# microsoft/DirectXTex

Measured on AMD Instinct MI355X. Metric: Mtexels/s BC7 encode (4096^2 RGBA8, TEX_COMPRESS_DEFAULT), higher is better.
Workload: dtype fp32 seed fit + i32 exact error sums (u8 texels in, 128-bit blocks out); 1 GPU; cfg2: 4096x4096 RGBA8 -> BC7_UNORM, TEX_COMPRESS_DEFAULT, one image per GPU, source and payload resident in HBM (dxtex_compress_device)

## Files before the change

### directxtex_amd/csrc/bc6h_encode.hip

```cpp
#include "dxtex_kernels.h"
#include "bc67_tables.h"
#include "bc7_core.h"
#include "bc6h_core.h"
#include "search_common.h"
#include <algorithm>
#include <cstdlib>
#include <cstdio>
#include <vector>

namespace dxtex
{
namespace
{
using namespace bc6h;

struct Ep16 { uint32_t a01, a2b0, b12; };
__device__ __forceinline__ Ep16 pack_ep16(const int (&A)[3], const int (&B)[3])
{
    Ep16 e;
    e.a01 = (uint32_t(A[0]) & 0xFFFFu) | (uint32_t(A[1]) << 16);
    e.a2b0 = (uint32_t(A[2]) & 0xFFFFu) | (uint32_t(B[0]) << 16);
    e.b12 = (uint32_t(B[1]) & 0xFFFFu) | (uint32_t(B[2]) << 16);
    return e;
}
// ... 973 lines not shown
        if (lane == 0) idx = atomicAdd(head, 1u);
        idx = uint32_t(__builtin_amdgcn_readfirstlane(int(idx)));
        if (idx >= live) break;
        const uint32_t myTask = a.order[idx].x;
        const Rec6 rec = a.recs[myTask];
        const uint32_t nb = myTask % a.nblocks;
        const int prec = a.prec1[myTask / a.nblocks];
        const float* gp = a.fpix + uint64_t(nb) * 48 + (lane & 15);
        const float tr = gp[0], tg = gp[16], tb = gp[32];
        EndPts e;
        unpack_ep16(rec.ep, sg, e.A, e.B);
        Perturb6 st = perturb6_begin(e, rec.err);
        while (st.ch < 3)
        {
            float err; int v;
            perturb6_wave_macro(tr, tg, tb, lane, st, prec, sg, err, v);
            st = perturb6_transition(st, err, v);
        }
        if (lane == 0)
        {
            a.recs[myTask].ep = pack_ep16(st.ep.A, st.ep.B);
            { const float mk = ep16_mark(sg, st.ep.A, st.ep.B); if (mk < 0.0f) a.recs[myTask].err = mk; }
        }
    }
}

__global__ void __launch_bounds__(256) bc6h_store_kernel(Bc6hArgs a)
{
    const uint32_t nb = blockIdx.x * 256u + threadIdx.x;
    if (nb >= a.nblocks) return;
    const Best6 b = a.best[nb];
    const BcSeg& im = seg_of(a.seg, nb);
    const uint32_t gb = im.nb0 + (nb - im.l0);
    const uint32_t by = gb / im.nbw, bx = gb - by * im.nbw;
    uint64_t* out = reinterpret_cast<uint64_t*>(im.dst + uint64_t(by) * im.dstRowPitch) + 2 * uint64_t(bx);
    out[0] = b.lo; out[1] = b.hi;
}

const uint64_t kMaxBlocksPerPass6 = dev_env("DXTEX_MAX_BLOCKS_PER_PASS") ? std::max<uint64_t>(1, strtoull(dev_env("DXTEX_MAX_BLOCKS_PER_PASS"), nullptr, 10)) : (1u << 22);
struct Scratch6
{
    size_t fpix, lists, seeds, recs, orgs, order, tinfo, counters, best, bounds, recs1, orgs1, order1, tinfo1, counters1, opts, total;
    explicit Scratch6(uint64_t nb)
    {
        auto up = [](size_t v) { return (v + 255) & ~size_t(255); };
        size_t o = 0;
        fpix = o; o = up(o + nb * 48 * sizeof(float));
        lists = o; o = up(o + nb * 8);
        seeds = o; o = up(o + nb * SEED_INTS * sizeof(int));
        recs = o; o = up(o + nb * 16 * sizeof(Rec6));
        orgs = o; o = up(o + nb * 16 * sizeof(OrgSave));
        order = o; o = up(o + nb * 16 * sizeof(uint2));
        tinfo = o; o = up(o + nb * 16 * sizeof(uint32_t));
        counters = o; o = up(o + 128 * sizeof(uint32_t));
        best = o; o = up(o + nb * sizeof(Best6));
        bounds = o; o = up(o + nb * 17 * sizeof(float));
        recs1 = o; o = up(o + nb * 4 * sizeof(Rec6));
        orgs1 = o; o = up(o + nb * 4 * sizeof(OrgSave));
        order1 = o; o = up(o + nb * 4 * sizeof(uint2));
        tinfo1 = o; o = up(o + nb * 4 * sizeof(uint32_t));
        counters1 = o; o = up(o + 128 * sizeof(uint32_t));
        opts = o; o = up(o + nb * 16 * sizeof(OptSave));
        total = o;
    }
};
}

size_t bc6h_scratch_bytes(uint64_t nblocks, size_t nimages)
{
    return Scratch6(nblocks < kMaxBlocksPerPass6 ? nblocks : kMaxBlocksPerPass6).total + seg_table_bytes(nblocks, kMaxBlocksPerPass6, nimages);
}

hipError_t launch_bc6h_encode(const SrcView& src, uint8_t* dst, uint64_t dstRowPitch, bool isSigned, void* scratch,
                              hipStream_t stream, KernelMarks* marks, const SideStreams* side)
{
    BcImage one; one.src = src; one.dst = dst; one.dstRowPitch = dstRowPitch;
    return launch_bc6h_encode_many(&one, 1, isSigned, scratch, stream, marks, side);
}

hipError_t launch_bc6h_encode_many(const BcImage* images, size_t count, bool isSigned, void* scratch, hipStream_t stream, KernelMarks* marks,
                                   const SideStreams* side)
{
#define DXTEX_MARK(NAME) do { if (marks) marks->mark(NAME); } while (0)
    std::vector<BcSeg> segs;
    std::vector<BcPass> passes;
    uint64_t perPass = 0;
    if (!build_passes(images, count, kMaxBlocksPerPass6, segs, passes, &perPass)) return hipSuccess;
    const Scratch6 L(perPass);
    uint8_t* base = static_cast<uint8_t*>(scratch);
    BcSeg* dSegs = reinterpret_cast<BcSeg*>(base + L.total);
    const hipError_t ce = upload_segments(dSegs, segs, passes, stream);
    if (ce != hipSuccess) return ce;
    for (const BcPass& pass : passes)
    {
        Bc6hArgs a;
        set_pass(a.seg, dSegs, segs, pass);
        a.nblocks = pass.nblocks;
        a.isSigned = isSigned ? 1 : 0;
        static const bool noPrune = dev_env("DXTEX_BC6H_NO_PRUNE") != nullptr;
        a.prune = noPrune ? 0 : 1;
        a.fpix = reinterpret_cast<float*>(base + L.fpix);
        a.lists = base + L.lists;
        a.seeds = reinterpret_cast<int*>(base + L.seeds);
        a.recs = reinterpret_cast<Rec6*>(base + L.recs);
        a.orgs = reinterpret_cast<OrgSave*>(base + L.orgs);
        a.order = reinterpret_cast<uint2*>(base + L.order);
        a.tinfo = reinterpret_cast<uint32_t*>(base + L.tinfo);
        a.counters = reinterpret_cast<uint32_t*>(base + L.counters);
        a.best = reinterpret_cast<Best6*>(base + L.best);
        a.bounds = reinterpret_cast<float*>(base + L.bounds);
        a.opts = reinterpret_cast<OptSave*>(base + L.opts);
        a.saveOpt = 0;
        a.boundsReady = 0;
        a.filterStats = 0;
        a.mode = ModeRt();

        DXTEX_MARK("bc6h_rough");
        hipLaunchKernelGGL(bc6h_rough_kernel, dim3((a.nblocks + 3) / 4), dim3(256), 0, stream, a);
        DXTEX_MARK("bc6h_block_seed");
        hipLaunchKernelGGL(bc6h_block_seed_kernel, dim3((a.nblocks + 255) / 256), dim3(256), 0, stream, a);
        if (dev_env("DXTEX_BC6H_DUMP"))
        {
            (void)hipStreamSynchronize(stream);
            const uint32_t n = std::min<uint32_t>(a.nblocks, 4);
            std::vector<uint8_t> l(n * 8); std::vector<int> sd(n * SEED_INTS);
            (void)hipMemcpy(l.data(), a.lists, l.size(), hipMemcpyDeviceToHost);
            (void)hipMemcpy(sd.data(), a.seeds, sd.size() * 4, hipMemcpyDeviceToHost);
            for (uint32_t b = 0; b < n; ++b)
            {
                fprintf(stderr, "block %u shapes:", b);
                for (int i = 0; i < 8; ++i) fprintf(stderr, " %d", l[b * 8 + i]);
                fprintf(stderr, "\n  seeds rank0:");
                for (int i = 0; i < 12; ++i) fprintf(stderr, " %d", sd[b * SEED_INTS + i]);
                fprintf(stderr, "\n");
            }
        }
        static const int onlyMode = dev_env("DXTEX_BC6H_ONLY_MODE") ? atoi(dev_env("DXTEX_BC6H_ONLY_MODE")) : -1;
        static const bool noSearch = dev_env("DXTEX_BC6H_NO_SEARCH") != nullptr;
        static const Bc6hMode kModes[14] = {
            { 0x00, 1, 1, 3, { 10, 10, 10 }, { 5, 5, 5 } }, { 0x01, 1, 1, 3, { 7, 7, 7 }, { 6, 6, 6 } }, { 0x02, 1, 1, 3, { 11, 11, 11 }, { 5, 4, 4 } },
            { 0x06, 1, 1, 3, { 11, 11, 11 }, { 4, 5, 4 } }, { 0x0a, 1, 1, 3, { 11, 11, 11 }, { 4, 4, 5 } }, { 0x0e, 1, 1, 3, { 9, 9, 9 }, { 5, 5, 5 } },
            { 0x12, 1, 1, 3, { 8, 8, 8 }, { 6, 5, 5 } }, { 0x16, 1, 1, 3, { 8, 8, 8 }, { 5, 6, 5 } }, { 0x1a, 1, 1, 3, { 8, 8, 8 }, { 5, 5, 6 } },
            { 0x1e, 1, 0, 3, { 6, 6, 6 }, { 6, 6, 6 } }, { 0x03, 0, 0, 4, { 10, 10, 10 }, { 10, 10, 10 } }, { 0x07, 0, 1, 4, { 11, 11, 11 }, { 9, 9, 9 } },
            { 0x0b, 0, 1, 4, { 12, 12, 12 }, { 8, 8, 8 } }, { 0x0f, 0, 1, 4, { 16, 16, 16 }, { 4, 4, 4 } } };
        auto set_mode_on = [&](Bc6hArgs& a, int mi)
        {
            const Bc6hMode& k = kModes[mi];
            a.mode.index = mi; a.mode.code = k.code; a.mode.regions2 = k.regions2; a.mode.transformed = k.transformed; a.mode.prec = k.prec[0];
            for (int c = 0; c < 3; ++c) a.mode.delta[c] = k.delta[c];
        };
        auto set_mode = [&](int mi) { set_mode_on(a, mi); };
        auto sort_tasks = [&](const Bc6hArgs& a, uint32_t ntasks, hipStream_t stream)
        {
            const uint32_t binGroups = std::min<uint32_t>(kBinGroups, (ntasks + 255) / 256);
            (void)hipMemsetAsync(a.counters, 0, 128 * sizeof(uint32_t), stream);
            hipLaunchKernelGGL(bc7_bin_count_kernel, dim3(binGroups), dim3(256), 0, stream, a.tinfo, ntasks, a.counters);
            hipLaunchKernelGGL(bc7_bin_scan_kernel, dim3(1), dim3(1), 0, stream, a.counters);
            hipLaunchKernelGGL(bc7_bin_scatter_kernel, dim3(binGroups), dim3(256), 0, stream, a.tinfo, ntasks, a.counters, a.order);
        };
        a.taskBase = 0;
        for (int m = 0; m < 4; ++m) a.prec1[m] = kModes[10 + m].prec[0];
        static const std::vector<int> order6 = []
        {
            std::vector<int> o;
            const char* e = dev_env("DXTEX_BC6H_ORDER");
            const char* p = e ? e : DXTEX_BC6H_DEFAULT_ORDER;
            while (*p) { if (*p >= '0' && *p <= '9') o.push_back(int(strtol(p, const_cast<char**>(&p), 10))); else ++p; }
            return o;
        }();
        int prevPrec = -1;
        a.samePrec = 0;
        std::vector<int> run2;
        for (int mi : order6) if (mi >= 0 && mi <= 9 && (onlyMode < 0 || mi == onlyMode)) run2.push_back(mi);
        static const int forkBack = dev_env("DXTEX_BC6H_FORK_BACK") ? atoi(dev_env("DXTEX_BC6H_FORK_BACK")) : 2;
        const SideStreams* fork = (marks || forkBack <= 0 || run2.size() < size_t(forkBack) + 1 || onlyMode >= 0) ? nullptr : side;
        Bc6hArgs a1 = a;
        a1.recs = reinterpret_cast<Rec6*>(base + L.recs1);
        a1.orgs = reinterpret_cast<OrgSave*>(base + L.orgs1);
        a1.order = reinterpret_cast<uint2*>(base + L.order1);
        a1.tinfo = reinterpret_cast<uint32_t*>(base + L.tinfo1);
        a1.counters = reinterpret_cast<uint32_t*>(base + L.counters1);
        a1.samePrec = 0;
        auto one_region_search = [&](hipStream_t stream, KernelMarks* marks)
        {
            const uint32_t gridPP = (a1.nblocks + 255) / 256;
            DXTEX_MARK("bc6h_pre_1region");
            a1.boundsReady = 0;
            for (int m = 0; m < 4; ++m)
            {
                if (onlyMode >= 0 && 10 + m != onlyMode) continue;
                set_mode_on(a1, 10 + m); a1.taskBase = uint32_t(m) * a1.nblocks;
                hipLaunchKernelGGL(bc6h_pre_kernel<0>, dim3(gridPP), dim3(256), 0, stream, a1);
                a1.boundsReady = 1;
            }
            const uint32_t ntasks = a1.nblocks * 4u;
            if (onlyMode >= 0)
                for (int m = 0; m < 4; ++m) if (10 + m != onlyMode) (void)hipMemsetAsync(a1.tinfo + uint64_t(m) * a1.nblocks, 0, uint64_t(a1.nblocks) * 4, stream);
            DXTEX_MARK("bc6h_bin_1region");
            sort_tasks(a1, ntasks, stream);
            DXTEX_MARK("bc6h_perturb_1region");
            static const uint32_t waveMax = dev_env("DXTEX_BC6H_WAVE_MAX") ? uint32_t(strtoul(dev_env("DXTEX_BC6H_WAVE_MAX"), nullptr, 0)) : kWaveTaskMax6;
            if (!noSearch)
            {
                hipLaunchKernelGGL(bc6h_perturb_kernel<16>, dim3(std::min<uint32_t>(kSearchWaves, (ntasks + 63) / 64)), dim3(64), 0, stream, a1, waveMax);
                hipLaunchKernelGGL(bc6h_perturb_wave_kernel, dim3(std::min<uint32_t>(kSearchWaves, ntasks)), dim3(64), 0, stream, a1, waveMax);
            }
        };
        bool forked = false;
        for (size_t at = 0; at < run2.size(); ++at)
        {
            const int mi = run2[at];
// ... 87 lines not shown
```

### directxtex_amd/csrc/bc7_encode.hip

```cpp
#include "dxtex_kernels.h"
#include "bc67_tables.h"
#include "bc7_core.h"
#include "search_common.h"
#include <algorithm>
#include <cstdio>
#include <cstdlib>
#include <vector>

namespace dxtex
{
namespace
{
using namespace bc7;

struct Cand { uint32_t err; uint32_t ord; uint64_t lo, hi; };

enum : int { SLOT_M0 = 0, SLOT_M1, SLOT_M2, SLOT_M3, SLOT_M4A, SLOT_M4B, SLOT_M5, SLOT_M6, SLOT_M7, NUM_SLOTS };
enum : int { LIST_BYTES = 64 };

enum : int { PHASE_ALL = 0, PHASE_EARLY = 1, PHASE_LATE = 2 };

struct Bc7Args
{
    SegTable seg;
// ... 1244 lines not shown
    const BcSeg& sg = seg_of(a.seg, i >> 4);
    load_block_texel(sg.src, sg.nbw, sg.nb0 + ((i >> 4) - sg.l0), i & 15u, f4, ldr);
    a.px[i] = ldr;
    if ((i & 15u) == 0) { a.zeroOrd[i >> 4] = 0xFFFFFFFFu; a.bestErr[i >> 4] = 0x7FFFFFFF; }
}

__global__ void __launch_bounds__(256) bc7_pick_kernel(Bc7Args a, uint32_t slotMask)
{
    const uint32_t nb = blockIdx.x * 256u + threadIdx.x;
    if (nb >= a.nblocks) return;
    const Cand* c = a.cands + uint64_t(nb) * NUM_SLOTS;
    uint64_t bestKey = ~0ull;
    uint64_t lo = 0, hi = 0;
#pragma unroll
    for (int s = 0; s < NUM_SLOTS; ++s)
    {
        if (!((slotMask >> s) & 1u)) continue;
        if (s == SLOT_M7 && a.flagged[1] == 0) continue;
        const Cand v = c[s];
        if (v.err == 0xFFFFFFFFu) continue;
        const uint64_t key = (uint64_t(v.err) << 32) | v.ord;
        if (key < bestKey) { bestKey = key; lo = v.lo; hi = v.hi; }
    }
    const BcSeg& sg = seg_of(a.seg, nb);
    const uint32_t gb = sg.nb0 + (nb - sg.l0);
    const uint32_t by = gb / sg.nbw, bx = gb - by * sg.nbw;
    uint64_t* out = reinterpret_cast<uint64_t*>(sg.dst + uint64_t(by) * sg.dstRowPitch) + 2 * uint64_t(bx);
    out[0] = lo; out[1] = hi;
}
}

namespace
{
const uint64_t kMaxBlocksPerPass = dev_env("DXTEX_MAX_BLOCKS_PER_PASS") ? std::max<uint64_t>(1, strtoull(dev_env("DXTEX_MAX_BLOCKS_PER_PASS"), nullptr, 10)) : (1u << 22);
constexpr int kMaxTasksPerBlock = 64;
const uint64_t kSmallPassBlocks = dev_env("DXTEX_BC7_SMALL_BLOCKS") ? strtoull(dev_env("DXTEX_BC7_SMALL_BLOCKS"), nullptr, 10) : 262144;
struct ScratchLayout
{
    size_t lists, cands, px, recs, order, tinfo, counters, zeroOrd, bestErr, seeds, seeds1, seeds3, flagcnt, auxRecs, auxOrder, auxTinfo, auxCounters, total;
    size_t auxTpb, auxSlices;
    explicit ScratchLayout(uint64_t nb, bool threeSubsets)
    {
        auto up = [](size_t v) { return (v + 255) & ~size_t(255); };
        const size_t tpb = threeSubsets ? kMaxTasksPerBlock : 32;
        const bool small = nb <= kSmallPassBlocks;
        auxTpb = small ? tpb : 4; auxSlices = small ? size_t(kSideStreams) : 2;
        size_t o = 0;
        lists = o; o = up(o + nb * LIST_BYTES);
        cands = o; o = up(o + nb * NUM_SLOTS * sizeof(Cand));
        px = o; o = up(o + nb * 64);
        recs = o; o = up(o + nb * tpb * sizeof(TaskRec));
        order = o; o = up(o + nb * tpb * sizeof(uint2));
        tinfo = o; o = up(o + nb * tpb * sizeof(uint32_t));
        counters = o; o = up(o + 64 * sizeof(uint32_t));
        zeroOrd = o; o = up(o + nb * sizeof(uint32_t));
        bestErr = o; o = up(o + nb * sizeof(int));
        seeds = o; o = up(o + nb * 64 * sizeof(uint2));
        seeds1 = o; o = up(o + nb * 2 * sizeof(uint2));
        seeds3 = o; o = up(o + (threeSubsets ? nb * 192 * sizeof(uint2) : 0));
        flagcnt = o; o = up(o + 256);
        auxRecs = o; o = up(o + auxSlices * nb * auxTpb * sizeof(TaskRec));
        auxOrder = o; o = up(o + auxSlices * nb * auxTpb * sizeof(uint2));
        auxTinfo = o; o = up(o + auxSlices * nb * auxTpb * sizeof(uint32_t));
        auxCounters = o; o = up(o + size_t(kSideStreams) * 64 * sizeof(uint32_t));
        total = o;
    }
};

template<int MODE, int IM>
void launch_mode(const Bc7Args& a0, hipStream_t stream, KernelMarks* marks, const char* const (&names)[7])
{
    typedef TaskMap<MODE, IM> TM;
    constexpr int BPW = (TM::TPB >= 64) ? 1 : 64 / TM::TPB;
    const uint32_t nb = a0.nblocks;
    const uint32_t ntasks = nb * uint32_t(TM::TPB);
    const uint32_t gridPP = (nb + 4 * BPW - 1) / (4 * BPW);
    constexpr bool kWhole = TM::NS == 1;
    constexpr uint32_t kExhMax = (MODE == 6) ? kWaveTaskMax : kWaveTaskMax45;
    static const bool noGroup = dev_env("DXTEX_BC7_NO_GROUP") != nullptr;
    const bool maybeShortP = kWhole && !noGroup && (MODE == 6 || ntasks <= 4u * kPerturbWaveMax);
    const bool maybeShortE = kWhole && !noGroup && (MODE == 6 || ntasks <= 4u * kExhMax);
    const uint32_t wavesP = std::min<uint32_t>(kSearchWaves, (ntasks + 1) / 2), wavesE = std::min<uint32_t>(kSearchWaves, ntasks);
    Bc7Args a = a0;
    a.gate = nullptr; a.gateMin = 0;
    if (a0.flagged && !(a0.flags & BCF_BC7_QUICK))
    {
        if (MODE == 7) { a.gate = a0.flagged + 1; a.gateMin = 1; }
        else if (a0.phase == PHASE_EARLY && (MODE == 4 || MODE == 5)) { a.gate = a0.flagged + 1; a.gateMin = std::max<uint32_t>(1u, a0.earlyAlphaMin); }
        else if (a0.phase == PHASE_EARLY && MODE == 6) { a.gate = a0.flagged; a.gateMin = std::max<uint32_t>(1u, a0.early6Min); }
    }
    a.perturbWaveMax = maybeShortP ? kPerturbWaveMax : 0u;
    a.exhWaveMax = maybeShortE ? kExhMax : 0u;
    if (marks) marks->mark(names[0]);
    hipLaunchKernelGGL((bc7_pre_kernel<MODE, IM>), dim3(gridPP), dim3(256), 0, stream, a);
    if (marks) marks->mark(names[1]);
    (void)hipMemsetAsync(a.counters, 0, 64 * sizeof(uint32_t), stream);
    const uint32_t binGroups = std::min<uint32_t>(kBinGroups, (ntasks + 255) / 256);
    hipLaunchKernelGGL(bc7_bin_count_kernel, dim3(binGroups), dim3(256), 0, stream, a.tinfo, ntasks, a.counters, a.gate, a.gateMin);
    hipLaunchKernelGGL(bc7_bin_scan_kernel, dim3(1), dim3(1), 0, stream, a.counters);
    hipLaunchKernelGGL(bc7_bin_scatter_kernel, dim3(binGroups), dim3(256), 0, stream, a.tinfo, ntasks, a.counters, a.order, a.gate, a.gateMin);
    if (marks) marks->mark(names[2]);
    const uint32_t waves = std::min<uint32_t>(kSearchWaves, (ntasks + 63) / 64);
    static const int tailBelow = dev_env("DXTEX_BC7_TAIL_BELOW") ? atoi(dev_env("DXTEX_BC7_TAIL_BELOW")) : 48;
    static const bool perturbPlain = dev_env("DXTEX_BC7_PERTURB_PLAIN") != nullptr;
    static const int rangeTests = dev_env("DXTEX_BC7_NO_PEEL") ? 3 : ((dev_env("DXTEX_BC7_RANGE_TESTS") ? atoi(dev_env("DXTEX_BC7_RANGE_TESTS")) & 0xFF : DXTEX_RANGE_TESTS) |
                                                                       ((dev_env("DXTEX_BC7_PEEL_LAYERS") ? atoi(dev_env("DXTEX_BC7_PEEL_LAYERS")) : 1) << 8));
    if constexpr (PaletteBits<MODE, IM>::AB == 0)
    {
        if constexpr (MODE == 1 || MODE == 6)
        {
            if (perturbPlain) hipLaunchKernelGGL((bc7_perturb_kernel<MODE, IM, CH_ALL>), dim3(waves), dim3(64), 0, stream, a, 0);
            else hipLaunchKernelGGL((bc7_perturb_filter_kernel<MODE, IM, CH_ALL>), dim3(waves), dim3(64), 0, stream, a, 0);
        }
        else
            hipLaunchKernelGGL((bc7_perturb_kernel<MODE, IM, CH_ALL>), dim3(waves), dim3(64), 0, stream, a, 0);
        if constexpr (kWhole) { if (maybeShortP) hipLaunchKernelGGL((bc7_perturb_wave_kernel<MODE, IM, CH_ALL>), dim3(wavesP), dim3(64), 0, stream, a); }
        if (marks) marks->mark(names[4]);
        if constexpr (kWhole) { if (maybeShortE) hipLaunchKernelGGL((bc7_exhaustive_wave_kernel<MODE, IM, CH_ALL>), dim3(wavesE), dim3(64), 0, stream, a); }
        hipLaunchKernelGGL((bc7_exhaustive_kernel<MODE, IM, CH_ALL>), dim3(waves), dim3(64), 0, stream, a, 1, tailBelow, rangeTests);
    }
    else
    {
        if constexpr (MODE == 4 && IM == 1 && DXTEX_PF_M4 != 0)
        {
            if (perturbPlain) hipLaunchKernelGGL((bc7_perturb_kernel<MODE, IM, CH_COLOR>), dim3(waves), dim3(64), 0, stream, a, 0);
            else hipLaunchKernelGGL((bc7_perturb_filter_kernel<MODE, IM, CH_COLOR>), dim3(waves), dim3(64), 0, stream, a, 0);
        }
        else
            hipLaunchKernelGGL((bc7_perturb_kernel<MODE, IM, CH_COLOR>), dim3(waves), dim3(64), 0, stream, a, 0);
        if (maybeShortP) hipLaunchKernelGGL((bc7_perturb_wave_kernel<MODE, IM, CH_COLOR>), dim3(wavesP), dim3(64), 0, stream, a);
        if (marks) marks->mark(names[3]);
        hipLaunchKernelGGL((bc7_perturb_kernel<MODE, IM, CH_ALPHA>), dim3(waves), dim3(64), 0, stream, a, 1);
        if (maybeShortP) hipLaunchKernelGGL((bc7_perturb_wave_kernel<MODE, IM, CH_ALPHA>), dim3(wavesP), dim3(64), 0, stream, a);
        if (marks) marks->mark(names[4]);
        if (maybeShortE) hipLaunchKernelGGL((bc7_exhaustive_wave_kernel<MODE, IM, CH_COLOR>), dim3(wavesE), dim3(64), 0, stream, a);
        hipLaunchKernelGGL((bc7_exhaustive_kernel<MODE, IM, CH_COLOR>), dim3(waves), dim3(64), 0, stream, a, 2, tailBelow, rangeTests);
        if (marks) marks->mark(names[5]);
        if (maybeShortE) hipLaunchKernelGGL((bc7_exhaustive_wave_kernel<MODE, IM, CH_ALPHA>), dim3(wavesE), dim3(64), 0, stream, a);
        hipLaunchKernelGGL((bc7_exhaustive_kernel<MODE, IM, CH_ALPHA>), dim3(waves), dim3(64), 0, stream, a, 3, tailBelow, rangeTests);
    }
    if (marks) marks->mark(names[6]);
    hipLaunchKernelGGL((bc7_post_kernel<MODE, IM>), dim3(gridPP), dim3(256), 0, stream, a);
#if defined(DXTEX_DEV)
    static const bool stats = dev_env("DXTEX_BC7_STATS") != nullptr;
    if (stats)
    {
        uint32_t c[40] = {};
        (void)hipStreamSynchronize(stream);
        (void)hipMemcpy(c, a.counters, sizeof(c), hipMemcpyDeviceToHost);
        std::fprintf(stderr, "bc7 stats %-22s phase %d: %9u task slots, %9u live; by size 16..1:", names[0], a.phase, ntasks, c[34]);
        for (int b = 16; b >= 1; --b) std::fprintf(stderr, " %u", c[b]);
        std::fprintf(stderr, "\n");
    }
// ... 146 lines not shown
            hipLaunchKernelGGL(bc7_texels_kernel, dim3((a.nblocks * 16 + 255) / 256), dim3(256), 0, stream, a);
        }
        DXTEX_MARK("bc7_block_seeds");
        if (!quick) hipLaunchKernelGGL(bc7_block_seeds_kernel<false>, dim3((a.nblocks + 255) / 256), dim3(256), 0, stream, a);
        hipLaunchKernelGGL(bc7_block_seeds_kernel<true>, dim3((a.nblocks + 255) / 256), dim3(256), 0, stream, a);
        static const std::vector<int> order = []
        {
            std::vector<int> o;
            const char* e = dev_env("DXTEX_BC7_ORDER");
            const char* p = e ? e : "16,7,14,18,15,0,1,2,3,24,28,25,26";
            while (*p)
            {
                if (*p >= '0' && *p <= '9') { o.push_back(int(strtol(p, const_cast<char**>(&p), 10))); }
                else ++p;
            }
            return o;
        }();
        a.phase = PHASE_ALL;
        if (quick) { DXTEX_MODE(6, 0, "mode6"); slotMask |= 1u << SLOT_M6; }
        auto run_step = [&](int step, Bc7Args a, hipStream_t stream, KernelMarks* marks)
        {
            a.phase = (step >= 20) ? PHASE_LATE : (step >= 10) ? PHASE_EARLY : PHASE_ALL;
            switch (step)
            {
            case 0: DXTEX_MODE(0, 0, "mode0"); slotMask |= 1u << SLOT_M0; break;
            case 1: DXTEX_MODE(1, 0, "mode1"); slotMask |= 1u << SLOT_M1; break;
            case 2: DXTEX_MODE(2, 0, "mode2"); slotMask |= 1u << SLOT_M2; break;
            case 3: DXTEX_MODE(3, 0, "mode3"); slotMask |= 1u << SLOT_M3; break;
            case 4: DXTEX_MODE(4, 0, "mode4_im0"); slotMask |= 1u << SLOT_M4A; break;
            case 14: DXTEX_MODE(4, 0, "mode4_im0_early"); slotMask |= 1u << SLOT_M4A; break;
            case 24: DXTEX_MODE(4, 0, "mode4_im0_late"); slotMask |= 1u << SLOT_M4A; break;
            case 8: DXTEX_MODE(4, 1, "mode4_im1"); slotMask |= 1u << SLOT_M4B; break;
            case 18: DXTEX_MODE(4, 1, "mode4_im1_early"); slotMask |= 1u << SLOT_M4B; break;
            case 28: DXTEX_MODE(4, 1, "mode4_im1_late"); slotMask |= 1u << SLOT_M4B; break;
            case 5: DXTEX_MODE(5, 0, "mode5"); slotMask |= 1u << SLOT_M5; break;
            case 15: DXTEX_MODE(5, 0, "mode5_early"); slotMask |= 1u << SLOT_M5; break;
            case 25: DXTEX_MODE(5, 0, "mode5_late"); slotMask |= 1u << SLOT_M5; break;
            case 6: DXTEX_MODE(6, 0, "mode6"); slotMask |= 1u << SLOT_M6; break;
            case 16: DXTEX_MODE(6, 0, "mode6_early"); slotMask |= 1u << SLOT_M6; break;
            case 26: DXTEX_MODE(6, 0, "mode6_late"); slotMask |= 1u << SLOT_M6; break;
            case 7: DXTEX_MODE(7, 0, "mode7"); slotMask |= 1u << SLOT_M7; break;
            default: break;
            }
        };
        auto family45 = [](int step) { const int m = step % 10; return m == 4 || m == 8 || m == 5; };
        static const bool serial45 = dev_env("DXTEX_BC7_SERIAL") != nullptr;
        const SideStreams* fork = (marks || serial45 || quick) ? nullptr : side;
        auto side_args = [&](const Bc7Args& a0, size_t k)
        {
            Bc7Args b = a0;
            b.recs = reinterpret_cast<TaskRec*>(base + L.auxRecs) + k * size_t(a0.nblocks) * L.auxTpb;
            b.order = reinterpret_cast<uint2*>(base + L.auxOrder) + k * size_t(a0.nblocks) * L.auxTpb;
            b.tinfo = reinterpret_cast<uint32_t*>(base + L.auxTinfo) + k * size_t(a0.nblocks) * L.auxTpb;
            b.counters = reinterpret_cast<uint32_t*>(base + L.auxCounters) + k * 64;
            return b;
        };
        static const std::vector<std::vector<std::vector<int>>> smallPlan = []
        {
            const char* e = dev_env("DXTEX_BC7_SMALL_PLAN");
            const char* p = e ? e : "1,26/3,2/16,14,15,18,7,0|24/28/25";
            std::vector<std::vector<std::vector<int>>> stages(1, std::vector<std::vector<int>>(1));
            while (*p)
            {
                if (*p >= '0' && *p <= '9') stages.back().back().push_back(int(strtol(p, const_cast<char**>(&p), 10)));
                else
                {
                    if (*p == '|') stages.emplace_back(1);
                    else if (*p == '/' && stages.back().size() < size_t(kSideStreams) + 1) stages.back().emplace_back();
                    ++p;
                }
            }
            return stages;
        }();
        static const bool noSmall = dev_env("DXTEX_BC7_NO_SMALL_PLAN") != nullptr;
        if (fork && !noSmall && smallPlanRuns)
        {
            for (const std::vector<std::vector<int>>& stage : smallPlan)
            {
                if (stage.size() > 1) (void)hipEventRecord(fork->forked, stream);
                for (size_t l = 1; l < stage.size(); ++l)
                {
                    hipStream_t s = fork->side[l - 1];
                    (void)hipStreamWaitEvent(s, fork->forked, 0);
                    const Bc7Args al = side_args(a, l - 1);
                    for (int step : stage[l])
                        if (three || (step != 0 && step != 2)) run_step(step, al, s, nullptr);
                    (void)hipEventRecord(fork->joined[l - 1], s);
                }
                for (int step : stage[0])
                    if (three || (step != 0 && step != 2)) run_step(step, a, stream, nullptr);
                for (size_t l = 1; l < stage.size(); ++l) (void)hipStreamWaitEvent(stream, fork->joined[l - 1], 0);
            }
        }
        else
        for (size_t at = 0; at < order.size() && !quick; )
        {
            const int step = order[at];
            if (!three && (step == 0 || step == 2)) { ++at; continue; }
            size_t run = 1;
            if (fork && family45(step))
                while (at + run < order.size() && run < 3 && family45(order[at + run]) && order[at + run] / 10 == step / 10) ++run;
            if (run == 1) { run_step(step, a, stream, marks); ++at; continue; }
            (void)hipEventRecord(fork->forked, stream);
            for (size_t k = 1; k < run; ++k)
            {
                const Bc7Args b = side_args(a, k - 1);
                (void)hipStreamWaitEvent(fork->side[k - 1], fork->forked, 0);
// ... 23 lines not shown
```

### directxtex_amd/csrc/search_common.h

```cpp
#pragma once
#include <hip/hip_runtime.h>
#include <stdint.h>
#include <algorithm>
#include <cstring>
#include <vector>
#include "dxtex_kernels.h"

namespace dxtex
{
namespace
{
struct BcSeg
{
    SrcView src;
    uint8_t* dst;
    uint64_t dstRowPitch;
    uint32_t nbw;
    uint32_t nb0;
    uint32_t l0;
    uint32_t pad;
};

struct SegTable
{
    BcSeg inl[2];
    const BcSeg* segs;
    uint32_t nseg;
};

__device__ __forceinline__ const BcSeg& seg_of(const SegTable& t, uint32_t local)
{
    if (t.nseg <= 2) return (t.nseg == 2 && t.inl[1].l0 <= local) ? t.inl[1] : t.inl[0];
    uint32_t lo = 0, hi = t.nseg;
    while (hi - lo > 1) { const uint32_t mid = (lo + hi) >> 1; if (t.segs[mid].l0 <= local) lo = mid; else hi = mid; }
    return t.segs[lo];
}

struct BcPass { uint32_t seg0, nseg, nblocks; };

inline uint64_t build_passes(const BcImage* images, size_t count, uint64_t maxPerPass, std::vector<BcSeg>& segs, std::vector<BcPass>& passes, uint64_t* perPassOut)
{
    uint64_t total = 0;
    for (size_t i = 0; i < count; ++i) total += uint64_t((images[i].src.width + 3) / 4) * ((images[i].src.height + 3) / 4);
    const uint64_t perPass = total < maxPerPass ? total : maxPerPass;
    *perPassOut = perPass;
    if (!total) return 0;
    BcPass cur = { 0, 0, 0 };
    for (size_t i = 0; i < count; ++i)
    {
        const uint32_t nbw = (images[i].src.width + 3) / 4, nbh = (images[i].src.height + 3) / 4;
        uint64_t left = uint64_t(nbw) * nbh, at = 0;
        while (left)
        {
            const uint64_t take = std::min<uint64_t>(left, perPass - cur.nblocks);
            BcSeg sg; sg.src = images[i].src; sg.dst = images[i].dst; sg.dstRowPitch = images[i].dstRowPitch;
            sg.nbw = nbw; sg.nb0 = uint32_t(at); sg.l0 = cur.nblocks; sg.pad = 0;
            segs.push_back(sg);
            ++cur.nseg; cur.nblocks += uint32_t(take); at += take; left -= take;
            if (cur.nblocks == perPass) { passes.push_back(cur); cur = { uint32_t(segs.size()), 0, 0 }; }
// ... 35 lines not shown
}

inline void set_pass(SegTable& t, const BcSeg* dSegs, const std::vector<BcSeg>& segs, const BcPass& pass)
{
    t.segs = dSegs + pass.seg0; t.nseg = pass.nseg;
    t.inl[0] = segs[pass.seg0]; t.inl[1] = segs[pass.seg0 + (pass.nseg > 1 ? 1 : 0)];
}

inline size_t seg_table_bytes(uint64_t nblocks, uint64_t maxPerPass, size_t nimages)
{
    const uint64_t perPass = nblocks < maxPerPass ? nblocks : maxPerPass;
    const uint64_t passes = perPass ? (nblocks + perPass - 1) / perPass : 1;
    return ((nimages + passes + 1) * sizeof(BcSeg) + 255) & ~size_t(255);
}

__device__ __forceinline__ void wave_lds_sync()
{
    __builtin_amdgcn_fence(__ATOMIC_RELEASE, "wavefront");
    __builtin_amdgcn_wave_barrier();
    __builtin_amdgcn_fence(__ATOMIC_ACQUIRE, "wavefront");
}

__device__ __forceinline__ int wave_prefix_min(int v)
{
    v = min(v, __builtin_amdgcn_update_dpp(v, v, 0x111, 0xF, 0xF, false));
    v = min(v, __builtin_amdgcn_update_dpp(v, v, 0x112, 0xF, 0xF, false));
    v = min(v, __builtin_amdgcn_update_dpp(v, v, 0x114, 0xF, 0xF, false));
    v = min(v, __builtin_amdgcn_update_dpp(v, v, 0x118, 0xF, 0xF, false));
    v = min(v, __builtin_amdgcn_update_dpp(v, v, 0x142, 0xA, 0xF, false));
    v = min(v, __builtin_amdgcn_update_dpp(v, v, 0x143, 0xC, 0xF, false));
    return v;
}

__device__ __forceinline__ void selection_pass(int& e, uint32_t& s, int lane, int i)
{
    const int v = (lane >= i) ? e : 0x7FFFFFFF;
    const int incl = wave_prefix_min(v);
    int excl = __builtin_amdgcn_update_dpp(0x7FFFFFFF, incl, 0x138, 0xF, 0xF, false);
    if (lane <= i) excl = 0x7FFFFFFF;
    const bool isrec = (lane > i) && (e < excl);
    const unsigned long long mask = __ballot(isrec);
    int srcLane = lane;
    if (isrec)
    {
        const unsigned long long below = mask & ((1ull << lane) - 1ull);
        srcLane = below ? (63 - __clzll(below)) : i;
    }
    else if (lane == i && mask)
        srcLane = 63 - __clzll(mask);
    e = __shfl(e, srcLane);
    s = uint32_t(__shfl(int(s), srcLane));
}

constexpr int kBinGroups = 2048;

__global__ void __launch_bounds__(256) bc7_bin_count_kernel(const uint32_t* tinfo, uint32_t ntasks, uint32_t* counters, const uint32_t* gate = nullptr, uint32_t gateMin = 0)
{
    if (gate && *gate < gateMin) return;
    __shared__ uint32_t hist[17];
    if (threadIdx.x < 17) hist[threadIdx.x] = 0;
    __syncthreads();
    const uint32_t per = (ntasks + gridDim.x - 1) / gridDim.x;
    const uint32_t t0 = blockIdx.x * per, t1 = min(ntasks, t0 + per);
    for (uint32_t t = t0 + threadIdx.x; t < t1; t += 256)
    {
        const uint32_t np = tinfo[t] >> 24;
        if (np) atomicAdd(&hist[np], 1u);
    }
    __syncthreads();
    if (threadIdx.x >= 1 && threadIdx.x <= 16 && hist[threadIdx.x]) atomicAdd(&counters[threadIdx.x], hist[threadIdx.x]);
}

__global__ void bc7_bin_scan_kernel(uint32_t* counters)
{
    if (threadIdx.x != 0 || blockIdx.x != 0) return;
    uint32_t run = 0;
    for (int b = 16; b >= 1; --b) { counters[17 + b] = run; run += counters[b]; }
    counters[34] = run;
}

__global__ void __launch_bounds__(256) bc7_bin_scatter_kernel(const uint32_t* tinfo, uint32_t ntasks, uint32_t* counters, uint2* order, const uint32_t* gate = nullptr, uint32_t gateMin = 0)
{
    if (gate && *gate < gateMin) return;
    __shared__ uint32_t hist[17], cursor[17];
    if (threadIdx.x < 17) hist[threadIdx.x] = 0;
    __syncthreads();
    const uint32_t per = (ntasks + gridDim.x - 1) / gridDim.x;
    const uint32_t t0 = blockIdx.x * per, t1 = min(ntasks, t0 + per);
    for (uint32_t t = t0 + threadIdx.x; t < t1; t += 256)
    {
        const uint32_t np = tinfo[t] >> 24;
        if (np) atomicAdd(&hist[np], 1u);
    }
    __syncthreads();
    if (threadIdx.x >= 1 && threadIdx.x <= 16)
        cursor[threadIdx.x] = hist[threadIdx.x] ? atomicAdd(&counters[17 + threadIdx.x], hist[threadIdx.x]) : 0u;
    __syncthreads();
    for (uint32_t t = t0 + threadIdx.x; t < t1; t += 256)
    {
        const uint32_t ti = tinfo[t], np = ti >> 24;
        if (np) order[atomicAdd(&cursor[np], 1u)] = make_uint2(t, ti);
    }
}

constexpr int kQueueBase = 36;
constexpr int kSearchWaves = 8192;

constexpr uint32_t kQueueBatch = 128;

struct WaveQueue
{
    uint32_t lo, hi;
    bool drained;
};

__device__ __forceinline__ uint32_t queue_take(WaveQueue& q, uint32_t* head, uint32_t live, unsigned long long idle, int lane)
{
    if (q.lo >= q.hi && !q.drained)
    {
        const uint32_t batch = (live > uint32_t(kSearchWaves) * 64u) ? kQueueBatch : 64u;
        uint32_t base = 0;
        if (lane == 0) base = atomicAdd(head, batch);
        base = uint32_t(__builtin_amdgcn_readfirstlane(int(base)));
        q.lo = base;
        q.hi = min(base + batch, live);
        if (base >= live) { q.drained = true; q.hi = q.lo; }
    }
    const uint32_t k = uint32_t(__popcll(idle & ((1ull << lane) - 1ull)));
    const uint32_t avail = q.hi - q.lo;
    const uint32_t mine = (((idle >> lane) & 1ull) && k < avail) ? (q.lo + k) : 0xFFFFFFFFu;
    q.lo += min(uint32_t(__popcll(idle)), avail);
    return mine;
}

}
}
```

Measured before the change: 136.5 Mtexels/s.

## Replace atomic bin sort with stable per-wave counting sort without scan kernel

The task bin sort now records per-workgroup and per-wave histograms in scratch. The scatter kernel derives each wave's start offsets by summing the histograms of earlier groups, which removes the separate single-thread scan launch. Shared-memory atomics in the scatter are replaced by wave ballots, so each lane's position in its bin comes from a popcount rank. The resulting order is stable and deterministic, which may give the later search passes more coherent memory access. In exchange, each scatter workgroup re-reads all earlier groups' histograms, which grows quadratically with group count, and the scratch area for histograms is larger.

Measured after the change: 137.1 Mtexels/s (median of 6 runs). About the same (+0.5%).

```diff
diff --git a/directxtex_amd/csrc/bc6h_encode.hip b/directxtex_amd/csrc/bc6h_encode.hip
--- a/directxtex_amd/csrc/bc6h_encode.hip
+++ b/directxtex_amd/csrc/bc6h_encode.hip
@@ -1049,14 +1049,14 @@
         orgs = o; o = up(o + nb * 16 * sizeof(OrgSave));
         order = o; o = up(o + nb * 16 * sizeof(uint2));
         tinfo = o; o = up(o + nb * 16 * sizeof(uint32_t));
-        counters = o; o = up(o + 128 * sizeof(uint32_t));
+        counters = o; o = up(o + (64 + kSortBlockWords) * sizeof(uint32_t));
         best = o; o = up(o + nb * sizeof(Best6));
         bounds = o; o = up(o + nb * 17 * sizeof(float));
         recs1 = o; o = up(o + nb * 4 * sizeof(Rec6));
         orgs1 = o; o = up(o + nb * 4 * sizeof(OrgSave));
         order1 = o; o = up(o + nb * 4 * sizeof(uint2));
         tinfo1 = o; o = up(o + nb * 4 * sizeof(uint32_t));
-        counters1 = o; o = up(o + 128 * sizeof(uint32_t));
+        counters1 = o; o = up(o + (64 + kSortBlockWords) * sizeof(uint32_t));
         opts = o; o = up(o + nb * 16 * sizeof(OptSave));
         total = o;
     }
@@ -1149,11 +1149,11 @@
         auto set_mode = [&](int mi) { set_mode_on(a, mi); };
         auto sort_tasks = [&](const Bc6hArgs& a, uint32_t ntasks, hipStream_t stream)
         {
-            const uint32_t binGroups = std::min<uint32_t>(kBinGroups, (ntasks + 255) / 256);
+            const uint32_t binGroups = sort_groups(ntasks);
+            uint32_t* wgHist = a.counters + 64 + kCounterWords;
             (void)hipMemsetAsync(a.counters, 0, 128 * sizeof(uint32_t), stream);
-            hipLaunchKernelGGL(bc7_bin_count_kernel, dim3(binGroups), dim3(256), 0, stream, a.tinfo, ntasks, a.counters);
-            hipLaunchKernelGGL(bc7_bin_scan_kernel, dim3(1), dim3(1), 0, stream, a.counters);
-            hipLaunchKernelGGL(bc7_bin_scatter_kernel, dim3(binGroups), dim3(256), 0, stream, a.tinfo, ntasks, a.counters, a.order);
+            hipLaunchKernelGGL(bc7_bin_count_kernel, dim3(binGroups), dim3(256), 0, stream, a.tinfo, ntasks, a.counters, wgHist);
+            hipLaunchKernelGGL(bc7_bin_scatter_kernel, dim3(binGroups), dim3(256), 0, stream, a.tinfo, ntasks, a.counters, wgHist, a.order);
         };
         a.taskBase = 0;
         for (int m = 0; m < 4; ++m) a.prec1[m] = kModes[10 + m].prec[0];
diff --git a/directxtex_amd/csrc/bc7_encode.hip b/directxtex_amd/csrc/bc7_encode.hip
--- a/directxtex_amd/csrc/bc7_encode.hip
+++ b/directxtex_amd/csrc/bc7_encode.hip
@@ -1320,7 +1320,7 @@
         recs = o; o = up(o + nb * tpb * sizeof(TaskRec));
         order = o; o = up(o + nb * tpb * sizeof(uint2));
         tinfo = o; o = up(o + nb * tpb * sizeof(uint32_t));
-        counters = o; o = up(o + 64 * sizeof(uint32_t));
+        counters = o; o = up(o + kSortBlockWords * sizeof(uint32_t));
         zeroOrd = o; o = up(o + nb * sizeof(uint32_t));
         bestErr = o; o = up(o + nb * sizeof(int));
         seeds = o; o = up(o + nb * 64 * sizeof(uint2));
@@ -1330,7 +1330,7 @@
         auxRecs = o; o = up(o + auxSlices * nb * auxTpb * sizeof(TaskRec));
         auxOrder = o; o = up(o + auxSlices * nb * auxTpb * sizeof(uint2));
         auxTinfo = o; o = up(o + auxSlices * nb * auxTpb * sizeof(uint32_t));
-        auxCounters = o; o = up(o + size_t(kSideStreams) * 64 * sizeof(uint32_t));
+        auxCounters = o; o = up(o + size_t(kSideStreams) * kSortBlockWords * sizeof(uint32_t));
         total = o;
     }
 };
@@ -1362,11 +1362,10 @@
     if (marks) marks->mark(names[0]);
     hipLaunchKernelGGL((bc7_pre_kernel<MODE, IM>), dim3(gridPP), dim3(256), 0, stream, a);
     if (marks) marks->mark(names[1]);
-    (void)hipMemsetAsync(a.counters, 0, 64 * sizeof(uint32_t), stream);
-    const uint32_t binGroups = std::min<uint32_t>(kBinGroups, (ntasks + 255) / 256);
-    hipLaunchKernelGGL(bc7_bin_count_kernel, dim3(binGroups), dim3(256), 0, stream, a.tinfo, ntasks, a.counters, a.gate, a.gateMin);
-    hipLaunchKernelGGL(bc7_bin_scan_kernel, dim3(1), dim3(1), 0, stream, a.counters);
-    hipLaunchKernelGGL(bc7_bin_scatter_kernel, dim3(binGroups), dim3(256), 0, stream, a.tinfo, ntasks, a.counters, a.order, a.gate, a.gateMin);
+    (void)hipMemsetAsync(a.counters, 0, kCounterWords * sizeof(uint32_t), stream);
+    const uint32_t binGroups = sort_groups(ntasks);
+    hipLaunchKernelGGL(bc7_bin_count_kernel, dim3(binGroups), dim3(256), 0, stream, a.tinfo, ntasks, a.counters, a.counters + kCounterWords, a.gate, a.gateMin);
+    hipLaunchKernelGGL(bc7_bin_scatter_kernel, dim3(binGroups), dim3(256), 0, stream, a.tinfo, ntasks, a.counters, a.counters + kCounterWords, a.order, a.gate, a.gateMin);
     if (marks) marks->mark(names[2]);
     const uint32_t waves = std::min<uint32_t>(kSearchWaves, (ntasks + 63) / 64);
     static const int tailBelow = dev_env("DXTEX_BC7_TAIL_BELOW") ? atoi(dev_env("DXTEX_BC7_TAIL_BELOW")) : 48;
@@ -1619,7 +1618,7 @@
             b.recs = reinterpret_cast<TaskRec*>(base + L.auxRecs) + k * size_t(a0.nblocks) * L.auxTpb;
             b.order = reinterpret_cast<uint2*>(base + L.auxOrder) + k * size_t(a0.nblocks) * L.auxTpb;
             b.tinfo = reinterpret_cast<uint32_t*>(base + L.auxTinfo) + k * size_t(a0.nblocks) * L.auxTpb;
-            b.counters = reinterpret_cast<uint32_t*>(base + L.auxCounters) + k * 64;
+            b.counters = reinterpret_cast<uint32_t*>(base + L.auxCounters) + k * size_t(kSortBlockWords);
             return b;
         };
         static const std::vector<std::vector<std::vector<int>>> smallPlan = []
diff --git a/directxtex_amd/csrc/search_common.h b/directxtex_amd/csrc/search_common.h
--- a/directxtex_amd/csrc/search_common.h
+++ b/directxtex_amd/csrc/search_common.h
@@ -5,6 +5,7 @@
 #include <cstring>
 #include <vector>
 #include "dxtex_kernels.h"
+#include "task_sort.h"
 
 namespace dxtex
 {
@@ -146,54 +147,83 @@
     s = uint32_t(__shfl(int(s), srcLane));
 }
 
-constexpr int kBinGroups = 2048;
-
-__global__ void __launch_bounds__(256) bc7_bin_count_kernel(const uint32_t* tinfo, uint32_t ntasks, uint32_t* counters, const uint32_t* gate = nullptr, uint32_t gateMin = 0)
+
+constexpr uint32_t kCounterWords = 64;
+constexpr uint32_t kSortBlockWords = kCounterWords + kSortHistWords;
+
+__global__ void __launch_bounds__(256) bc7_bin_count_kernel(const uint32_t* tinfo, uint32_t ntasks, uint32_t* counters, uint32_t* wgHist, const uint32_t* gate = nullptr, uint32_t gateMin = 0)
 {
     if (gate && *gate < gateMin) return;
-    __shared__ uint32_t hist[17];
-    if (threadIdx.x < 17) hist[threadIdx.x] = 0;
-    __syncthreads();
-    const uint32_t per = (ntasks + gridDim.x - 1) / gridDim.x;
-    const uint32_t t0 = blockIdx.x * per, t1 = min(ntasks, t0 + per);
-    for (uint32_t t = t0 + threadIdx.x; t < t1; t += 256)
-    {
-        const uint32_t np = tinfo[t] >> 24;
-        if (np) atomicAdd(&hist[np], 1u);
-    }
-    __syncthreads();
-    if (threadIdx.x >= 1 && threadIdx.x <= 16 && hist[threadIdx.x]) atomicAdd(&counters[threadIdx.x], hist[threadIdx.x]);
-}
-
-__global__ void bc7_bin_scan_kernel(uint32_t* counters)
-{
-    if (threadIdx.x != 0 || blockIdx.x != 0) return;
-    uint32_t run = 0;
-    for (int b = 16; b >= 1; --b) { counters[17 + b] = run; run += counters[b]; }
-    counters[34] = run;
-}
-
-__global__ void __launch_bounds__(256) bc7_bin_scatter_kernel(const uint32_t* tinfo, uint32_t ntasks, uint32_t* counters, uint2* order, const uint32_t* gate = nullptr, uint32_t gateMin = 0)
+    __shared__ uint32_t hist[kSortWaves][kSortBins + 1];
+    if (threadIdx.x < kSortWaves * (kSortBins + 1)) (&hist[0][0])[threadIdx.x] = 0;
+    __syncthreads();
+    const uint32_t wave = threadIdx.x >> 6, lane = threadIdx.x & 63;
+    const SortSlice ws = sort_wave_slice(sort_group_slice(ntasks, gridDim.x, blockIdx.x), wave);
+    for (uint32_t t = ws.t0 + lane; t < ws.t1; t += 64)
+    {
+        const uint32_t np = sort_bin_of(tinfo[t]);
+        if (np) atomicAdd(&hist[wave][np], 1u);
+    }
+    __syncthreads();
+    if (threadIdx.x < kSortWaves * kSortBins)
+        wgHist[kSortWaveRows + blockIdx.x * uint32_t(kSortWaves * kSortBins) + threadIdx.x] = hist[threadIdx.x >> 4][(threadIdx.x & 15) + 1];
+    if (threadIdx.x < kSortBins)
+    {
+        uint32_t total = 0;
+        for (int w = 0; w < kSortWaves; ++w) total += hist[w][threadIdx.x + 1];
+        wgHist[blockIdx.x * uint32_t(kSortBins) + threadIdx.x] = total;
+        if (total) atomicAdd(&counters[threadIdx.x + 1], total);
+    }
+}
+
+__device__ __forceinline__ void sort_wave_step(uint32_t t, uint32_t ti, uint32_t& cur, uint32_t lane, uint2* order, uint32_t ntasks)
+{
+    const uint32_t np = sort_bin_of(ti);
+    unsigned long long todo = __ballot(np != 0);
+    while (todo)
+    {
+        const uint32_t b = uint32_t(__builtin_amdgcn_readlane(int(np), int(sort_next_lane(todo))));
+        const unsigned long long m = __ballot(np == b);
+        const uint32_t pos = uint32_t(__builtin_amdgcn_readlane(int(cur), int(b) - 1)) + sort_rank(m, lane);
+        if (np == b && pos < ntasks) order[pos] = make_uint2(t, ti);
+        if (lane == b - 1) cur += sort_count(m);
+        todo &= ~m;
+    }
+}
+
+__global__ void __launch_bounds__(256) bc7_bin_scatter_kernel(const uint32_t* tinfo, uint32_t ntasks, uint32_t* counters, const uint32_t* wgHist, uint2* order, const uint32_t* gate = nullptr, uint32_t gateMin = 0)
 {
     if (gate && *gate < gateMin) return;
-    __shared__ uint32_t hist[17], cursor[17];
-    if (threadIdx.x < 17) hist[threadIdx.x] = 0;
-    __syncthreads();
-    const uint32_t per = (ntasks + gridDim.x - 1) / gridDim.x;
-    const uint32_t t0 = blockIdx.x * per, t1 = min(ntasks, t0 + per);
-    for (uint32_t t = t0 + threadIdx.x; t < t1; t += 256)
-    {
-        const uint32_t np = tinfo[t] >> 24;
-        if (np) atomicAdd(&hist[np], 1u);
-    }
-    __syncthreads();
-    if (threadIdx.x >= 1 && threadIdx.x <= 16)
-        cursor[threadIdx.x] = hist[threadIdx.x] ? atomicAdd(&counters[17 + threadIdx.x], hist[threadIdx.x]) : 0u;
-    __syncthreads();
-    for (uint32_t t = t0 + threadIdx.x; t < t1; t += 256)
-    {
-        const uint32_t ti = tinfo[t], np = ti >> 24;
-        if (np) order[atomicAdd(&cursor[np], 1u)] = make_uint2(t, ti);
+    __shared__ uint32_t part[256];
+    __shared__ uint32_t start[kSortWaves][kSortBins];
+    const uint32_t tid = threadIdx.x, g = blockIdx.x;
+    uint32_t sum = 0;
+    for (uint32_t r = tid >> 4; r < g; r += 16) sum += wgHist[r * uint32_t(kSortBins) + (tid & 15)];
+    part[tid] = sum;
+    __syncthreads();
+    if (tid < kSortBins)
+    {
+        uint32_t counts[kSortBins + 1];
+        counts[0] = 0;
+        for (int b = 1; b <= kSortBins; ++b) counts[b] = counters[b];
+        uint32_t at = sort_bin_base(counts, tid + 1);
+        for (int r = 0; r < 16; ++r) at += part[r * 16 + tid];
+        const uint32_t* waves = wgHist + kSortWaveRows + g * uint32_t(kSortWaves * kSortBins);
+        for (int w = 0; w < kSortWaves; ++w) { start[w][tid] = at; at += waves[w * kSortBins + tid]; }
+        if (g == 0 && tid == 0) counters[34] = sort_live_total(counts);
+    }
+    __syncthreads();
+    const uint32_t wave = uint32_t(__builtin_amdgcn_readfirstlane(int(tid >> 6))), lane = tid & 63;
+    const SortSlice ws = sort_wave_slice(sort_group_slice(ntasks, gridDim.x, g), wave);
+    const uint32_t trips = sort_wave_trips(ws);
+    uint32_t cur = lane < kSortBins ? start[wave][lane] : 0u;
+    for (uint32_t i = 0; i < trips; i += 2)
+    {
+        const uint32_t ta = ws.t0 + i * 64u + lane, tb = ta + 64u;
+        const uint32_t ia = ta < ws.t1 ? tinfo[ta] : 0u;
+        const uint32_t ib = tb < ws.t1 ? tinfo[tb] : 0u;
+        sort_wave_step(ta, ia, cur, lane, order, ntasks);
+        sort_wave_step(tb, ib, cur, lane, order, ntasks);
     }
 }
 
diff --git a/directxtex_amd/csrc/task_sort.h b/directxtex_amd/csrc/task_sort.h
--- /dev/null
+++ b/directxtex_amd/csrc/task_sort.h
@@ -0,0 +1,58 @@
+#pragma once
+#include <stdint.h>
+
+#if defined(__HIPCC__)
+#define DXTEX_SORT_FN __host__ __device__ inline
+#else
+#define DXTEX_SORT_FN inline
+#endif
+
+namespace dxtex
+{
+constexpr int kBinGroups = 2048;
+constexpr int kSortBins = 16;
+constexpr int kSortWaves = 4;
+constexpr uint32_t kSortWaveRows = uint32_t(kBinGroups) * kSortBins;
+constexpr uint32_t kSortHistWords = uint32_t(kBinGroups) * kSortBins * (1 + kSortWaves);
+
+struct SortSlice { uint32_t t0, t1; };
+
+DXTEX_SORT_FN uint32_t sort_min(uint32_t a, uint32_t b) { return a < b ? a : b; }
+
+DXTEX_SORT_FN uint32_t sort_groups(uint32_t ntasks) { return sort_min(uint32_t(kBinGroups), (ntasks + 255u) / 256u); }
+
+DXTEX_SORT_FN uint32_t sort_bin_of(uint32_t tinfo) { const uint32_t b = tinfo >> 24; return b <= uint32_t(kSortBins) ? b : 0u; }
+
+DXTEX_SORT_FN SortSlice sort_group_slice(uint32_t ntasks, uint32_t groups, uint32_t g)
+{
+    const uint32_t per = (ntasks + groups - 1u) / groups;
+    const uint64_t at = uint64_t(g) * per;
+    SortSlice s;
+    s.t0 = at < ntasks ? uint32_t(at) : ntasks;
+    s.t1 = sort_min(ntasks - s.t0, per) + s.t0;
+    return s;
+}
+
+DXTEX_SORT_FN SortSlice sort_wave_slice(SortSlice g, uint32_t w)
+{
+    const uint32_t n = g.t1 - g.t0, per = (n + uint32_t(kSortWaves) - 1u) / uint32_t(kSortWaves);
+    SortSlice s;
+    s.t0 = g.t0 + sort_min(n, w * per);
+    s.t1 = s.t0 + sort_min(g.t1 - s.t0, per);
+    return s;
+}
+
+DXTEX_SORT_FN uint32_t sort_wave_trips(SortSlice w) { return (w.t1 - w.t0 + 63u) / 64u; }
+
+DXTEX_SORT_FN uint32_t sort_bin_base(const uint32_t* counts, uint32_t b)
+{
+    uint32_t base = 0;
+    for (uint32_t bb = 1; bb <= uint32_t(kSortBins); ++bb) if (bb > b) base += counts[bb];
+    return base;
+}
+DXTEX_SORT_FN uint32_t sort_live_total(const uint32_t* counts) { return sort_bin_base(counts, 0); }
+
+DXTEX_SORT_FN uint32_t sort_rank(unsigned long long mask, uint32_t lane) { return uint32_t(__builtin_popcountll(mask & ((1ull << lane) - 1ull))); }
+DXTEX_SORT_FN uint32_t sort_count(unsigned long long mask) { return uint32_t(__builtin_popcountll(mask)); }
+DXTEX_SORT_FN uint32_t sort_next_lane(unsigned long long todo) { return uint32_t(__builtin_ctzll(todo)); }
+}
```
